# synthesizer-project/synference

Measured on AMD Instinct MI355X. Metric: posterior samples/sec (accepted, prior-box rejection included), higher is better.
Workload: dtype f32

## Files before the change

include/synference_hip.h:

```cpp
#ifndef SYNFERENCE_HIP_H
#define SYNFERENCE_HIP_H

#include <stddef.h>
#include <stdint.h>

#ifdef __cplusplus
extern "C" {
#endif

typedef struct sf_flow sf_flow;
typedef struct sf_opt sf_opt;

enum sf_status {
  SF_OK = 0,
  SF_ERR_INVALID = -1,
  SF_ERR_HIP = -2,
  SF_ERR_NO_DEVICE = -3,
  SF_ERR_STATE = -4
};

enum sf_kind { SF_MAF = 0, SF_NSF = 1, SF_NSF_AR = 2, SF_MAF_AR = 3 };

typedef struct sf_flow_desc {
  int32_t kind;
// ... 46 lines not shown

int sf_flow_log_prob_grad(sf_flow* f, const float* theta , const float* x, int64_t rows_per_x, int64_t B,
                          float* lp , float* dtheta , void* stream);

int sf_map_step(int64_t B, int64_t D, float* phi , float* exp_avg , float* exp_avg_sq ,
                float* theta , const float* lp , const float* g_theta , const float* lo ,
                const float* hi , float* best_theta , float* best_lp , float learning_rate,
                int64_t step, int save_best, void* stream);

int sf_flow_inverse_from_noise(sf_flow* f, const float* z , const float* x ,
                               int64_t B, float* theta , float* logdet ,
                               void* stream);
int sf_flow_inverse_from_noise_sampler(sf_flow* f, const float* z , const float* x , int64_t B,
                                       float* theta , void* stream);
int sf_set_sampler_fp32(int on);

int sf_flow_sample_round(sf_flow* f, const float* x , int64_t S,
                         const uint32_t* slots, int64_t slot_base, int64_t n_slots,
                         uint32_t attempt, int32_t attempts_per_slot, uint64_t seed, uint32_t stream_id,
                         const float* lo , const float* hi ,
                         float* out , uint32_t* rejected, uint32_t* n_rejected,
                         int32_t* n_drawn, void* stream);

int sf_flow_prepare_context(sf_flow* f, const float* x , int64_t M, void* stream);
int sf_flow_release_context(sf_flow* f);

int sf_flow_sample(sf_flow* f, const float* x , int64_t M, int64_t S,
                   const float* lo, const float* hi, uint64_t seed, int32_t max_attempts,
                   float* out , int32_t* n_drawn , int64_t* n_unfilled ,
                   void* stream);
// ... 188 lines not shown
```

synference_amd/_lib.py:

```python
from __future__ import annotations

import ctypes as C
import os
from pathlib import Path

_HERE = Path(__file__).resolve().parent
LIB_PATH = _HERE / "lib" / "libsynference_hip.so"

c_f32p = C.POINTER(C.c_float)
c_i32p = C.POINTER(C.c_int32)
c_u32p = C.POINTER(C.c_uint32)


class sf_flow_desc(C.Structure):
    _fields_ = [
        ("kind", C.c_int32), ("D", C.c_int32), ("C", C.c_int32), ("H", C.c_int32),
        ("T", C.c_int32), ("K", C.c_int32), ("NB", C.c_int32), ("scale_fn", C.c_int32),
        ("hidden_bf16", C.c_int32),
        ("tail_bound", C.c_float), ("min_bin_width", C.c_float), ("min_bin_height", C.c_float),
        ("min_derivative", C.c_float), ("maf_eps", C.c_float), ("lu_eps", C.c_float),
        ("theta_mean", c_f32p), ("theta_std", c_f32p), ("x_mean", c_f32p), ("x_std", c_f32p),
        ("perms", c_i32p), ("ar_slope", C.c_float),
    ]

# ... 40 lines not shown
                                    C.c_void_p, C.c_void_p, C.c_void_p]),
    "sf_scatter_empirical": (C.c_int, [C.c_void_p, C.c_int64, C.c_int32, C.POINTER(sf_noise_band), c_f32p, C.c_int64, C.c_int32,
                                       C.c_uint64, C.c_void_p, C.c_void_p, C.c_void_p]),
    "sf_apply_scalings": (C.c_int, [C.c_void_p, C.c_void_p, C.c_int64, C.c_int32, C.POINTER(sf_noise_band), c_f32p, C.c_int64,
                                    C.c_void_p, C.c_void_p, C.c_void_p]),
    "sf_pit_ranks": (C.c_int, [C.c_void_p, C.c_void_p, C.c_int64, C.c_int64, C.c_int32, C.c_void_p, C.c_void_p]),
    "sf_tarp_coverage": (C.c_int, [C.c_void_p, C.c_void_p, C.c_int64, C.c_int64, C.c_int32, C.c_void_p, C.c_int32, C.c_int32,
                                   C.c_int32, C.c_int32, C.c_uint64, C.c_void_p, C.c_void_p, C.c_void_p, C.c_void_p,
                                   C.c_void_p]),
    "sf_copy_to_host_f64": (C.c_int, [C.c_void_p, C.c_void_p, C.c_int64, C.c_void_p]),
    "sf_flow_packed16_size": (C.c_int64, [C.c_void_p]),
    "sf_flow_pack_table16": (C.c_int, [C.c_void_p, C.c_void_p, C.c_void_p, C.c_int64]),
    "sf_flow_packed16b_size": (C.c_int64, [C.c_void_p]),
    "sf_flow_inverse_from_noise_sampler": (C.c_int, [C.c_void_p, C.c_void_p, C.c_void_p, C.c_int64, C.c_void_p, C.c_void_p]),
    "sf_set_sampler_fp32": (C.c_int, [C.c_int]),
    "sf_flow_set_sample_row_offset": (C.c_int, [C.c_void_p, C.c_int64]),
    "sf_flow_train_path": (C.c_int, [C.c_void_p, C.c_int64, C.c_int]),
    "sf_flow_trainc_size": (C.c_int64, [C.c_void_p]),
    "sf_flow_trainc_grad_size": (C.c_int64, [C.c_void_p]),
    "sf_flow_cst_size": (C.c_int64, [C.c_void_p]),
    "sf_flow_trainc_table": (C.c_int, [C.c_void_p, C.c_void_p, C.c_void_p, C.c_int64, C.c_void_p, C.c_int64, C.c_void_p,
                                       C.c_void_p, C.c_int64]),
    "sf_flow_pack_table16b": (C.c_int, [C.c_void_p, C.c_void_p, C.c_int64]),
    "sf_flow_get_params": (C.c_int, [C.c_void_p, C.c_void_p, C.c_int64, C.c_int, C.c_void_p]),
    "sf_flow_prepare_context": (C.c_int, [C.c_void_p, C.c_void_p, C.c_int64, C.c_void_p]),
    "sf_flow_release_context": (C.c_int, [C.c_void_p]),
    "sf_flow_sample": (C.c_int, [C.c_void_p, C.c_void_p, C.c_int64, C.c_int64, C.c_void_p, C.c_void_p,
                                 C.c_uint64, C.c_int32, C.c_void_p, C.c_void_p, C.POINTER(C.c_int64),
                                 C.c_void_p]),
    "sf_flow_sample_slots": (C.c_int, [C.c_void_p, C.c_void_p, C.c_int64, C.c_int64, C.c_void_p, C.c_int64, C.c_void_p,
# ... 94 lines not shown
```

synference_amd/csrc/sf_api.hip:

```cpp
#include <hip/hip_runtime.h>

#include <chrono>
#include <cmath>
#include <cstdio>
#include <cstdlib>
#include <cstring>
#include <string>
#include <vector>

#include "sf_internal.h"
#include "sf_train.h"
#include "sf_nsf1.h"
#include "sf_nsfar.h"
#include "sf_nsfc.h"
#include "sf_trainc.h"

namespace {
thread_local std::string g_err;

int hip_fail(hipError_t e, const char* what) {
  return sf_fail(SF_ERR_HIP, std::string(what) + ": " + hipGetErrorString(e));
}
}

// ... 195 lines not shown
  add("o_wg0", v.o_wg[0]); add("o_bg0", v.o_bg[0]); add("o_w10", v.o_w1[0]); add("o_b10", v.o_b1[0]);
  add("o_w20", v.o_w2[0]); add("o_b20", v.o_b2[0]); add("o_wg1", v.o_wg[1]); add("o_bg1", v.o_bg[1]);
  add("o_w11", v.o_w1[1]); add("o_b11", v.o_b1[1]); add("o_w21", v.o_w2[1]); add("o_b21", v.o_b2[1]);
  add("o_wout", v.o_wout); add("o_bout", v.o_bout); add("o_lu", v.o_lu);
  add("c_pscale", v.c_pscale); add("c_pshift", v.c_pshift); add("c_tdim", v.c_tdim);
  add("c_xmean", v.c_xmean); add("c_xstd", v.c_xstd); add("c_dslot", v.c_dslot);
  add("nsf_split_sampler", f->L.nsfS.ok); add("trainc_ok", f->L.trc.ok); add("nsfc_ok", f->L.nsc.ok);
  add("inc_ok", v.inc_ok); add("hidden_bf16", v.hidden_bf16); add("tB_stride", v.tB_stride); add("n_parts", v.n_parts); add("part_max", v.part_max);
  add("n_params", f->L.n_params); add("n_packed", f->L.n_packed);
  {
    int R = 0, NV = 0;
    SfDev vv = v;
    vv.packed16 = reinterpret_cast<const float*>(1);
    sf_ctab_shape(vv, R, NV);
    add("ctab_floats_per_galaxy", (long)v.T * NV * R);
  }
  add("o16_w0", v.o16_w0); add("o16_wc", v.o16_wc); add("o16_b0", v.o16_b0); add("o16_wk0", v.o16_wk[0]);
  add("o16_wk1", v.o16_wk[1]); add("o16_bk0", v.o16_bk[0]); add("o16_bk1", v.o16_bk[1]); add("o16_hv", v.o16_hv);
  add("o16_hvb", v.o16_hvb); add("o16_wh", v.o16_wh); add("o16_bh", v.o16_bh); add("o16_wp", v.o16_wp); add("t16_a_tab", v.t16_a_tab);
  add("t16_a", v.t16_a); add("t16B_stride", v.t16B_stride); add("nP16", v.nP16); add("o16B_wk0", v.o16B_wk[0]); add("o16B_wk1", v.o16B_wk[1]);
  add("m16_ok", v.m16_ok); add("m16_span", v.m16_span); add("nT16", v.nT16); add("nC16", v.nC16); add("t16_stride", v.t16_stride);
  s += "\"g16_tile\": [";
  for (int i = 0; i < SF_DMAX; ++i) s += std::to_string(v.g16_tile[i]) + (i + 1 < SF_DMAX ? ", " : "], ");
  s += "\"g16_lo\": [";
  for (int i = 0; i < SF_DMAX; ++i) s += std::to_string(v.g16_lo[i]) + (i + 1 < SF_DMAX ? ", " : "], ");
  s += "\"g_kend\": [";
  for (int i = 0; i < SF_DMAX; ++i) s += std::to_string(v.g_kend[i]) + (i + 1 < SF_DMAX ? ", " : "], ");
  s += "\"g_lo\": [";
  for (int i = 0; i < SF_DMAX; ++i) s += std::to_string(v.g_lo[i]) + (i + 1 < SF_DMAX ? ", " : "], ");
  s += "\"g_tile\": [";
// ... 143 lines not shown
extern "C++" {
static int g_sampler_fp32 = -2;
void sf_sampler_fp32_set(int on) { g_sampler_fp32 = on < 0 ? -1 : (on ? 1 : 0); }
int sf_sampler_fp32_get() {
  if (g_sampler_fp32 == -2) { const char* e = std::getenv("SF_SAMPLER_FP32"); g_sampler_fp32 = (e && *e) ? (std::atoi(e) != 0 ? 1 : 0) : -1; }
  return g_sampler_fp32;
}
int sf_sampler_fp32_for(int kind) {
  const int g = sf_sampler_fp32_get();
  return g < 0 ? (kind == SF_MAF ? 1 : 0) : g;
}
}
int sf_set_sampler_fp32(int on) {
  sf_sampler_fp32_set(on);
  return SF_OK;
}

int sf_flow_train_path(const sf_flow* f, int64_t B, int want_dctx) {
  if (!f) return sf_fail(SF_ERR_INVALID, "null handle");
  if (f->nsf1) return 4;
  if (f->nsfar) return 5;
  if (B > 0 && sf_trainc_eligible(f->L, want_dctx != 0)) return sf_trainc_groups((long)B, &f->L.trc, f->L.dev.T);
  if (B > 0 && sf_nsfc_eligible(f->L, want_dctx != 0)) return 3;
  return 0;
}

static void seed_keys(uint64_t seed, uint32_t stream_id, uint32_t& k0, uint32_t& k1) {
  k0 = (uint32_t)(seed & 0xffffffffu);
  k1 = (uint32_t)(seed >> 32) ^ stream_id;
}
// ... 642 lines not shown
```

synference_amd/csrc/sf_internal.h:

```cpp
#pragma once
#include <hip/hip_runtime.h>
#include <stdint.h>

#include "sf_buf.h"
#include "sf_layout.h"
#include "sf_queue.h"

struct SfSampleArgsHost {
  const float* x = nullptr;
  const float* z_in = nullptr;
  long S = 1;
  const uint32_t* slots = nullptr;
  long slot_base = 0;
  long n_items = 0;
  uint32_t attempt = 0, k0 = 0, k1 = 0;
  unsigned long long rng_slot_offset = 0;
  int attempts_per_slot = 1;
  int log2_attempts = 0;
  const float* lo = nullptr;
  const float* hi = nullptr;
  float* out = nullptr;
  int out_f64 = 0;
  float* logdet_out = nullptr;
  uint32_t* rejected = nullptr;
// ... 33 lines not shown
void sf_sampler_fp32_set(int on);
int sf_sampler_fp32_get();
int sf_sampler_fp32_for(int kind);
void sf_ctab_shape(const SfDev& m, int& R, int& NV);
hipError_t sf_launch_ctab(const SfDev& m, const float* x, long M, float* tab, hipStream_t st);
hipError_t sf_launch_maf_ctab16(const SfDev& m, const float* x, long M, float* tab, hipStream_t st);
hipError_t sf_launch_maf_fuse16(const SfDev& m, hipStream_t st);
struct SfMaf16Plan {
  bool ok16 = false;
  bool sampler16 = false;
  bool fp32 = false;
  bool span = false;
  bool head_mfma = false;
  int dd = 0;
  bool fused = false;
};
SfMaf16Plan sf_maf16_plan(const SfDev& m);
hipError_t sf_launch_maf_find16_zin(const SfDev& m, const SfSampleArgsHost& a, hipStream_t st);
hipError_t sf_launch_pack(const float* flat, const int32_t* s1, const int32_t* s2, float* packed, long n,
                          hipStream_t st);
hipError_t sf_launch_pack_bf16(const float* flat, const int32_t* src, unsigned short* out, long n, hipStream_t st);
hipError_t sf_launch_pack_bf16_split(const float* flat, const int32_t* src, unsigned short* out, long n, hipStream_t st);
hipError_t sf_launch_fill_nan_rows(float* out, const uint32_t* slots, long n, int D, hipStream_t st, int out_f64 = 0);
hipError_t sf_launch_fill_i32(int32_t* p, long n, int32_t v, hipStream_t st);
hipError_t sf_launch_exclusive_scan_i32(const int32_t* cnt, int n, int32_t* offs, int32_t* total, hipStream_t st);
hipError_t sf_launch_account_window(const uint32_t* list, const uint32_t* best, long n, long S, uint32_t a_lo, uint32_t A,
                                    int32_t* n_drawn, int32_t* gal_acc, hipStream_t st);
hipError_t sf_launch_filter_survivors(uint32_t* list, unsigned int* n_surv, long S, const int32_t* gal_acc, float* out,
                                      int D, hipStream_t st, int out_f64 = 0);

#include <string>
#define SF_MAX_DEVICES 16
// ... 138 lines not shown
```

synference_amd/csrc/sf_maf16.hip:

```cpp
#include "sf_maf16_pass.h"

template <int NB, bool SPAN>
__global__ __launch_bounds__(256, 3) void k_maf_inv16(SfDev m, SfSampleArgsHost a) {
  const int lane = threadIdx.x & 63, wave = threadIdx.x >> 6;
  const int s = lane & 15, g4 = lane >> 4;
  const long item = ((long)blockIdx.x * 4 + wave) * 16 + s;
  const bool valid = item < a.n_items;
  const long it = valid ? item : a.n_items - 1;
  const SfItem16 I = sf_item16(m, a, it, g4);
  f32x4 u = I.u;
  const uint32_t slot = I.slot, att_mine = I.att;
  const long gal = I.gal, ps_idx = I.ps;
  const float* xr = a.x + gal * m.C;
  float logdet = 0.f;

  const float* ctg = (m.ctab && !a.z_in) ? m.ctab + (size_t)gal * m.T * m.ctab_R : nullptr;
  f32x4 ct0;
  if (!ctg) ct0 = sf_ctx_tile16(m, xr, 0, g4);

  const int NT = m.nT16;
  SfPass16 S;
#pragma unroll
  for (int k = 0; k < 3; ++k)
#pragma unroll
// ... 120 lines not shown
  static constexpr int oB_wk1 = entries * 512, B_stride = (NB * entries * 512 + 1023) / 1024 * 1024;
  static bool matches(const SfDev& m) {
    return m.nT16 == NT && m.o16_w0 == o_w0 && m.o16_b0 == o_b0 && m.o16_bk[0] == o_bk0 && (NB < 2 || m.o16_bk[1] == o_bk1) &&
           m.o16_hv == o_hv && m.o16_hvb == o_hvb && m.o16_wh == o_wh && m.o16_bh == o_bh && m.o16_wp == o_wp && m.t16_a_tab == a_tab &&
           m.o16B_wk[0] == 0 && (NB < 2 || m.o16B_wk[1] == oB_wk1) && m.t16B_stride == B_stride;
  }
  static __device__ __forceinline__ void apply(SfDev& m) {
    m.nT16 = NT; m.o16_w0 = o_w0; m.o16_b0 = o_b0; m.o16_bk[0] = o_bk0; m.o16_bk[1] = o_bk1; m.o16_hv = o_hv; m.o16_hvb = o_hvb;
    m.o16_wh = o_wh; m.o16_bh = o_bh; m.o16_wp = o_wp; m.t16_a_tab = a_tab; m.o16B_wk[0] = 0; m.o16B_wk[1] = oB_wk1; m.t16B_stride = B_stride;
  }
};

#ifndef SF_SAMP16_WG_FUSED
#define SF_SAMP16_WG_FUSED 4
#endif
template <int NB, bool SPAN, bool HM, int DD = 0, int PREC = 0>
__global__ __launch_bounds__(256, (SPAN ? 3 : (PREC == 2 ? SF_SAMP16_WG_FUSED : 4))) void k_maf_samp16(SfSamp16Args args_in) {
  static_assert(DD == 0 || (HM && !SPAN && DD >= 2 && DD <= 5), "unrolled passes: head tile, aligned placement, D <= 5");
  using HID = SfHid16<PREC>;
  constexpr int TPW = SF_SAMP16_TPW;
  constexpr int IPW = 64 * TPW;
  const int wave = threadIdx.x >> 6;
  unsigned int* ctrl = reinterpret_cast<unsigned int*>(
      sf_lds16 + (args_in.m.ctab ? args_in.m.t16_a_tab : args_in.m.t16_a) + HID::lds_floats(args_in.m, !SPAN));
  unsigned int pf;
  sf_q_begin<IPW>(args_in.a, ctrl, pf);
  float* ecb = reinterpret_cast<float*>(ctrl + SF_Q_WORDS(IPW));
  sf_ecb16_build<true>(ecb, args_in.m, args_in.a);
#ifdef SF_Q_STATS
  const unsigned long long qs_k0 = __builtin_amdgcn_s_memtime();
  unsigned long long qs_iters = 0, qs_last_work = 0;
  unsigned long long qs_ph[10] = {0, 0, 0, 0, 0, 0, 0, 0, 0, 0};
  if (threadIdx.x == 0) atomicMin(&args_in.a.q->stats[10], __builtin_amdgcn_s_memrealtime());
#endif
  for (;;) {
    const SfSamp16Args* ap;
    {
      auto kp = __builtin_amdgcn_kernarg_segment_ptr();
      asm volatile("" : "+s"(kp));
      ap = (const SfSamp16Args*)kp;
    }
    const SfDev& m_arg = ap->m;
    SfDev m_fix;
    if constexpr (DD > 0) { m_fix = m_arg; SfFix16<NB, DD>::apply(m_fix); }
    const SfDev& m = DD > 0 ? m_fix : m_arg;
    const SfSampleArgsHost& a = ap->a;
    const int lane = (threadIdx.x & 63) + sf_opaque_zero();
    const int s = lane & 15, g4 = lane >> 4;
#ifdef SF_Q_STATS
    const unsigned long long qs_t_top = __builtin_amdgcn_s_memrealtime();
#endif
    if (!sf_q_fetch<IPW, 64>(a, ctrl, pf)) {
#ifdef SF_Q_STATS
      if (threadIdx.x == 0) {
        for (int i = 0; i < 10; ++i) atomicAdd(&a.q->stats[14 + i], qs_ph[i]);
        atomicAdd(&a.q->stats[9], __builtin_amdgcn_s_memtime() - qs_k0);
        atomicMax(&a.q->stats[11], qs_iters);
        atomicMax(&a.q->stats[12], qs_last_work);
        atomicMax(&a.q->stats[13], __builtin_amdgcn_s_memrealtime());
      }
#endif
      break;
    }
#ifdef SF_Q_STATS
    if (a.qtrace && threadIdx.x == 0 && qs_iters < (2048u * 256u) / gridDim.x) {
      uint32_t* tr = a.qtrace + ((size_t)blockIdx.x * ((2048u * 256u) / gridDim.x) + qs_iters) * 4;
      tr[0] = (uint32_t)__builtin_amdgcn_s_memrealtime(); tr[1] = ctrl[0]; tr[2] = ctrl[1] | (ctrl[9] << 8);
    }
    ++qs_iters;
    const unsigned long long qs_t_fetch = __builtin_amdgcn_s_memrealtime();
    const int qs_o = ctrl[9] ? 5 : 0;
    qs_ph[qs_o + 0] += qs_t_fetch - qs_t_top;
    unsigned long long qs_t_mark = qs_t_fetch;
#endif
    const int NT = m.nT16;
    const unsigned int n_items = ctrl[0] << ctrl[1];
    f32x4 u_t[TPW];
    unsigned int g_t[TPW];
    f32x4& u_cur = u_t[0];
    unsigned int& gal_cur = g_t[0];
#pragma unroll
    for (int j = TPW - 1; j >= 0; --j) {
      const int wi = (j * 4 + wave) * 16 + s;
      const unsigned int n_ent = ctrl[0];
      const int lgA = (int)ctrl[1];
      const unsigned int e = (unsigned)wi >> lgA;
      const unsigned int ee = e < n_ent ? e : 0u;
      const uint32_t slot = ctrl[SF_Q_HDR + ee];
      const uint32_t att = ctrl[SF_Q_HDR + IPW + ee] + ((unsigned)wi & ((1u << lgA) - 1u));
      float z4[4];
      sf_normal4(a.k0, a.k1, (uint64_t)slot + a.rng_slot_offset, att, (uint32_t)g4, z4);
#pragma unroll
      for (int r = 0; r < 4; ++r) u_t[j][r] = (4 * g4 + r < m.D) ? z4[r] : 0.f;
      g_t[j] = slot / (uint32_t)a.S;
    }
    SfTiles16 tiles;
    if constexpr (DD == 0) tiles.pack(m);
    typename HID::State S;
    S.tab = DD > 0 ? true : m.ctab != nullptr;
    for (int t = m.T - 1; t >= 0; --t) {
      const int dsl = (int)m.cst[m.c_dslot + t * SF_DMAX + s];
      S.c0p = S.tab ? m.ctab + ((size_t)gal_cur * m.T + t) * m.ctab_R + (PREC == 2 ? m.nT16 * 16 : 0) : nullptr;
      if constexpr (PREC == 2) sf_pre16g_load<DD - 1>(S, g4);
      else if (HM && S.tab) sf_c0_prefetch(S, tiles.tile(2), g4);
#ifdef SF_Q_STATS
      { const unsigned long long n = __builtin_amdgcn_s_memrealtime(); qs_ph[qs_o + (t == m.T - 1 ? 1 : 3)] += n - qs_t_mark; qs_t_mark = n; }
#endif
      __syncthreads();
      sf_stage16<PREC, !SPAN>(m, t, S.tab ? m.t16_a_tab : m.t16_a, wave);
      __syncthreads();
#ifdef SF_Q_STATS
      { const unsigned long long n = __builtin_amdgcn_s_memrealtime(); qs_ph[qs_o + 2] += n - qs_t_mark; qs_t_mark = n; }
#endif
      const float* tp = sf_lds16;
      const void* tpB = sf_lds16 + (S.tab ? m.t16_a_tab : m.t16_a);
#pragma unroll 1
      for (int j = 0; j < TPW; ++j) {
        const bool tile_has_work = (unsigned)((j * 4 + wave) * 16) < n_items;
        if (tile_has_work) {
          if (j > 0) {
            S.c0p = S.tab ? m.ctab + ((size_t)gal_cur * m.T + t) * m.ctab_R + (PREC == 2 ? m.nT16 * 16 : 0) : nullptr;
            if constexpr (PREC == 2) sf_pre16g_load<DD - 1>(S, g4);
            else if (HM && S.tab) sf_c0_prefetch(S, tiles.tile(2), g4);
          }
          if (HM) S.hdone = sf_ld4(tp + m.o16_bh + g4 * 4);
          if constexpr (PREC == 2) {
            float* scr = (float*)tpB + HID::blk_floats(m) + wave * SF_G16_SCR + s * SF_G16_ROW;
            sf_transform16g<NB, DD>(m, tp, static_cast<const float*>(tpB), S, dsl, u_cur, scr, lane, g4);
          } else {
            S.xr = a.x + gal_cur * m.C;
            if constexpr (DD > 0) {
              sf_transform16s<HID, NB, DD>(m, tp, tpB, S, NT, dsl, u_cur, lane, g4);
            } else {
              HID::template clear<false, HM>(S);
#pragma unroll
              for (int r = 0; r < 4; ++r) S.ut[r] = 0.f;
              {
                const int sl = __builtin_amdgcn_readlane(dsl, 0);
                sf_pass16_deg1(m, tp, S.ut, sl, sf_slot16_own(u_cur, sl), g4);
              }
              for (int p = 2; p <= m.D; ++p) {
                const int sl = __builtin_amdgcn_readlane(dsl, p - 1);
// ... 6 lines not shown
        if (TPW > 1) {
          const f32x4 tu = u_t[0];
          const unsigned int tg = g_t[0];
#pragma unroll
          for (int q = 0; q + 1 < TPW; ++q) { u_t[q] = u_t[q + 1]; g_t[q] = g_t[q + 1]; }
          u_t[TPW - 1] = tu;
          g_t[TPW - 1] = tg;
        }
      }
    }
#ifdef SF_Q_STATS
    { const unsigned long long n = __builtin_amdgcn_s_memrealtime(); qs_ph[qs_o + 3] += n - qs_t_mark; qs_t_mark = n; }
#endif
#pragma unroll 1
    for (int j = 0; j < TPW; ++j) {
      const int wi = (j * 4 + wave) * 16 + s;
      const unsigned int n_ent = ctrl[0];
      const int lgA = (int)ctrl[1];
      const unsigned int e = (unsigned)wi >> lgA;
      const bool entry_ok = e < n_ent;
      const unsigned int ee = entry_ok ? e : 0u;
      const uint32_t slot = ctrl[SF_Q_HDR + ee];
      const uint32_t att_base = ctrl[SF_Q_HDR + IPW + ee];
      const uint32_t att = att_base + ((unsigned)wi & ((1u << lgA) - 1u));
      const bool valid = entry_ok && att < a.attempt_limit;
      float th[4];
      int tdc[4];
      const uint32_t acc16 = sf_accept16(sf_theta_box16(ecb, u_cur, g4, th, tdc), valid);
      const int A = 1 << lgA;
      int first, me;
      if (lgA <= 4) {
        const int grp0 = (s / A) * A;
        const uint32_t gmask = (acc16 >> grp0) & ((1u << A) - 1u);
        first = gmask ? (int)__builtin_ctz(gmask) : -1;
        me = s - grp0;
      } else {
        if ((threadIdx.x & 63) == 0) ctrl[20 + wave] = acc16 ? (unsigned)__builtin_ctz(acc16) : 16u;
        __syncthreads();
        const int gw0 = (int)(((e << lgA) >> 4) & 3u), gwn = A >> 4;
        first = -1;
#pragma unroll
        for (int w = 3; w >= 0; --w) {
          const unsigned int cw = ctrl[20 + w];
          if (w >= gw0 && w < gw0 + gwn && cw < 16u) first = (w - gw0) * 16 + (int)cw;
        }
        me = wi - (int)(e << lgA);
        if (TPW > 1) __syncthreads();
      }
      if (lgA == 0) {
        const int Dn = DD > 0 ? DD : m.D;
// ... 44 lines not shown
      }
      if (TPW > 1) {
        const f32x4 tu = u_t[0];
#pragma unroll
        for (int q = 0; q + 1 < TPW; ++q) u_t[q] = u_t[q + 1];
        u_t[TPW - 1] = tu;
      }
    }
#ifdef SF_Q_STATS
    qs_last_work = __builtin_amdgcn_s_memrealtime();
    qs_ph[qs_o + 4] += qs_last_work - qs_t_mark;
    if (a.qtrace && threadIdx.x == 0 && qs_iters <= (2048u * 256u) / gridDim.x)
      a.qtrace[((size_t)blockIdx.x * ((2048u * 256u) / gridDim.x) + qs_iters - 1) * 4 + 3] = (uint32_t)qs_last_work;
#endif
  }
}

template <int NB, int DD, int PREC = 0>
__global__ __launch_bounds__(256, 4) void k_maf_find16s(SfDev m, SfSampleArgsHost a) {
  using HID = SfHid16<PREC>;
  SfFix16<NB, DD>::apply(m);
  const int lane = threadIdx.x & 63, wave = threadIdx.x >> 6;
  const int s = lane & 15, g4 = lane >> 4;
  float* ecb = sf_lds16 + m.t16_a_tab + HID::lds_floats(m, true);
  sf_ecb16_build<false>(ecb, m, a);
  const int NT = m.nT16;
  f32x4 u_cur, u_oth;
  long gal_cur = 0, gal_oth = 0;
#pragma unroll
  for (int j = 1; j >= 0; --j) {
// ... 118 lines not shown
    if (m.g16_tile[p - 1] != p - 2) return 0;
  bool fits = false;
  if (m.NB == 1) fits = m.D == 3 ? SfFix16<1, 3>::matches(m) : (m.D == 4 ? SfFix16<1, 4>::matches(m) : SfFix16<1, 5>::matches(m));
  else if (m.NB == 2) fits = m.D == 3 ? SfFix16<2, 3>::matches(m) : (m.D == 4 ? SfFix16<2, 4>::matches(m) : SfFix16<2, 5>::matches(m));
  return fits ? m.D : 0;
}
SfMaf16Plan sf_maf16_plan(const SfDev& m) {
  SfMaf16Plan pl;
  pl.fp32 = sf_sampler_fp32_for(SF_MAF) != 0;
  pl.ok16 = m.kind == SF_MAF && m.m16_ok && !m.hidden_bf16 && m.packed16 != nullptr;
  pl.sampler16 = pl.ok16 && (m.packed16B != nullptr || pl.fp32);
  pl.span = m.m16_span != 0;
  pl.head_mfma = !m.m16_span && m.o16_wh >= 0;
  pl.dd = pl.head_mfma ? sf_maf16_seq_d(m) : 0;
  pl.fused = pl.dd > 0 && pl.fp32 && m.o16_wp >= 0 && m.ctab_R == 2 * m.nT16 * 16;
  return pl;
}

template <int NB, int DD, int PREC>
static hipError_t sf_launch_find16s(const SfDev& m, const SfSampleArgsHost& a, hipStream_t st) {
  static SfAttrCache attr;
  const size_t sh = ((size_t)m.t16_a_tab + (size_t)SfHid16<PREC>::lds_floats(m, true)) * sizeof(float) + 80 * sizeof(float);
  if (hipError_t e = sf_lds_optin16(k_maf_find16s<NB, DD, PREC>, attr); e != hipSuccess) return e;
  hipLaunchKernelGGL((k_maf_find16s<NB, DD, PREC>), dim3((unsigned)((a.n_items + 127) / 128)), dim3(256), sh, st, m, a);
  return hipGetLastError();
}

template <int NB, bool SPAN, bool HM, int PREC = 0>
__global__ __launch_bounds__(256, 3) void k_maf_inv16b(SfDev m, const float* __restrict__ z, const float* __restrict__ x,
                                                       long n, float* __restrict__ out) {
  using HID = SfHid16<PREC>;
// ... 128 lines not shown
  }
}
hipError_t sf_launch_maf_fuse16(const SfDev& m, hipStream_t st) {
  hipLaunchKernelGGL(k_maf_fuse16, dim3((unsigned)m.T), dim3(256), 0, st, m);
  return hipGetLastError();
}
hipError_t sf_launch_maf_ctab16(const SfDev& m, const float* x, long M, float* tab, hipStream_t st) {
  hipLaunchKernelGGL(k_maf_ctab16, dim3((unsigned)((M + 63) / 64), (unsigned)m.T), dim3(256), 0, st, m, x, M, tab);
  return hipGetLastError();
}

bool sf_maf16_enabled(const SfDev& m, const SfSampleArgsHost& a) {
  return sf_maf16_plan(m).ok16 && (a.attempts_per_slot <= 16 || a.best != nullptr);
}

static int sf_resident_blocks16(const void* fn, size_t sh, int cap) {
  int dev = 0, cus = 256, per = cap;
  if (hipGetDevice(&dev) == hipSuccess) {
    hipDeviceProp_t pr;
    if (hipGetDeviceProperties(&pr, dev) == hipSuccess && pr.multiProcessorCount > 0) cus = pr.multiProcessorCount;
  }
  int occ = 0;
  if (hipOccupancyMaxActiveBlocksPerMultiprocessor(&occ, fn, 256, sh) == hipSuccess && occ > 0) per = occ < cap ? occ : cap;
  return cus * per;
}

template <int NB, bool SPAN, bool HM, int DD, int PREC>
static hipError_t sf_launch16q_p(const SfDev& m, const SfSampleArgsHost& a, hipStream_t st) {
  static SfAttrCache attr;
  static SfResidentCache rcache;
  const size_t sh = ((size_t)(m.ctab ? m.t16_a_tab : m.t16_a) + (size_t)SfHid16<PREC>::lds_floats(m, !SPAN)) * sizeof(float) +
                    (SF_Q_WORDS(64 * SF_SAMP16_TPW) + 96) * sizeof(unsigned int);
  if (sh > 160 * 1024) return hipErrorInvalidValue;
  if (hipError_t e = sf_lds_optin16(k_maf_samp16<NB, SPAN, HM, DD, PREC>, attr); e != hipSuccess) return e;
  int resident = 0, cur_dev = 0;
  (void)hipGetDevice(&cur_dev);
  if (!rcache.get(cur_dev, sh, resident)) {
    resident = sf_resident_blocks16((const void*)k_maf_samp16<NB, SPAN, HM, DD, PREC>, sh, SPAN ? 3 : (PREC == 2 ? SF_SAMP16_WG_FUSED : 4));
    rcache.put(cur_dev, sh, resident);
  }
  long grid = (a.n_items + 64 * SF_SAMP16_TPW - 1) / (64 * SF_SAMP16_TPW);
  if (grid > resident) grid = resident;
  SfSamp16Args args;
  args.m = m;
  args.a = a;
  hipLaunchKernelGGL((k_maf_samp16<NB, SPAN, HM, DD, PREC>), dim3((unsigned)grid), dim3(256), sh, st, args);
  return hipGetLastError();
}
template <int NB, bool SPAN, bool HM, int DD>
static hipError_t sf_launch16q(const SfDev& m, const SfSampleArgsHost& a, const SfMaf16Plan& pl, hipStream_t st) {
  if constexpr (DD > 0) {
    if (pl.fused) return sf_launch16q_p<NB, SPAN, HM, DD, 2>(m, a, st);
  }
  if (pl.fp32) return sf_launch16q_p<NB, SPAN, HM, DD, 1>(m, a, st);
  if (!m.packed16B) return hipErrorInvalidValue;
  return sf_launch16q_p<NB, SPAN, HM, DD, 0>(m, a, st);
}
template <int NB, bool SPAN>
static hipError_t sf_launch16(const SfDev& m, const SfSampleArgsHost& a, hipStream_t st) {
  static SfAttrCache attr;
  const size_t sh = (size_t)m.t16_stride * sizeof(float);
  if (hipError_t e = sf_lds_optin16(k_maf_inv16<NB, SPAN>, attr); e != hipSuccess) return e;
  const long per_block = 4L * 16;
  hipLaunchKernelGGL((k_maf_inv16<NB, SPAN>), dim3((unsigned)((a.n_items + per_block - 1) / per_block)), dim3(256), sh, st, m, a);
  return hipGetLastError();
// ... 23 lines not shown
```

synference_amd/csrc/sf_maf16_pass.h:

```cpp
#pragma once
#include <hip/hip_runtime.h>

#include <type_traits>

#include "sf_device.h"
#include "sf_internal.h"
#include "sf_rng.h"

typedef float f32x4 __attribute__((ext_vector_type(4)));
typedef float f32x2 __attribute__((ext_vector_type(2)));
#define SF_MFMA16(a, b, c) __builtin_amdgcn_mfma_f32_16x16x4f32((a), (b), (c), 0, 0, 0)

__device__ __forceinline__ float sf_sum4groups(float v) {
  v += __shfl_xor(v, 16, 64);
  v += __shfl_xor(v, 32, 64);
  return v;
}
__device__ __forceinline__ f32x4 sf_mma16(float4 w, const f32x4& in, f32x4 acc) {
  acc = SF_MFMA16(w.x, in[0], acc);
  acc = SF_MFMA16(w.y, in[1], acc);
  acc = SF_MFMA16(w.z, in[2], acc);
  acc = SF_MFMA16(w.w, in[3], acc);
  return acc;
}
// ... 651 lines not shown
    const int NT = m.nT16, nb = m.NB < 2 ? m.NB : 2;
    const int per = CP ? NT * (NT + 1) / 2 : NT * NT;
    constexpr int K0 = PREC == 2 ? 1 : 0;
    float4* __restrict__ dF = d4 + (a_floats >> 2);
    for (int e = __builtin_amdgcn_readfirstlane(wave); e < (nb - K0) * per; e += 4) {
      const int k = K0 + (e >= per ? 1 : 0), ee = e - (k - K0) * per;
      int src_blk = ee;
      if (CP) {
        const int ot = ee >= 6 ? 3 : (ee >= 3 ? 2 : (ee >= 1 ? 1 : 0));
        src_blk = ot * NT + (ee - ot * (ot + 1) / 2);
      }
      const int owk = k ? m.o16_wk[1] : m.o16_wk[0];
      const float4* g = sa + ((owk >> 2) + src_blk * 64) + lane_;
      __builtin_amdgcn_global_load_lds((const void*)g, (void __attribute__((address_space(3)))*)(dF + e * 64), 16, 0, 0);
    }
  }
  __builtin_amdgcn_s_waitcnt(0x0f70);
}

struct SfHid16Plain {
  using State = SfPass16;
  template <int OT, int NB, bool CP, bool HM>
  static __device__ __forceinline__ void pass(const SfDev& m, const float* tp, const void*, State& S, int NT, int sl, float u_sl,
                                              int lane, int g4, int) {
    sf_pass16<OT, NB>(m, tp, S, NT, sl, u_sl, lane, g4);
  }
  template <int LO, int HI, int NB>
  static __device__ __forceinline__ void span(const SfDev& m, const float* tp, const void*, State& S, int NT, int sl, float u_sl,
                                              int lane, int g4) {
    sf_pass16_span<LO, HI, NB>(m, tp, S, NT, sl, u_sl, lane, g4);
// ... 109 lines not shown
```

synference_amd/csrc/sf_queue.h:

```cpp
#pragma once
#include <hip/hip_runtime.h>
#include <stdint.h>

struct SfQueue {
  unsigned int dense_next; unsigned int _p0[31];
  unsigned int head;       unsigned int _p1[31];
  unsigned int reserve;    unsigned int _p2[31];
  unsigned int resolved;   unsigned int _p3[31];
  unsigned int n_surv;     unsigned int dropped;
  unsigned int _p4[30];
  unsigned int error;      unsigned int _p5[31];
  unsigned int rej0;       unsigned int _p6[31];
  unsigned long long evals; unsigned int _p7[30];
  unsigned long long stats[24];
};

#define SF_Q_SPIN_TICKS 1500000000ull
#define SF_Q_SPIN_ITERS 4000000u

#define SF_Q_HDR 24
#define SF_Q_WORDS(IPW) (SF_Q_HDR + 5 * (IPW))

__device__ __forceinline__ unsigned int sf_q_ld(const unsigned int* p) {
  return __hip_atomic_load(p, __ATOMIC_RELAXED, __HIP_MEMORY_SCOPE_AGENT);
}

#ifdef __HIPCC__
#ifdef SF_Q_STATS
#define SF_QS_T() __builtin_amdgcn_s_memtime()
#define SF_QS_ADD(i, v) do { if (threadIdx.x == 0) atomicAdd(&a.q->stats[i], (unsigned long long)(v)); } while (0)
#else
#define SF_QS_T() 0ull
#define SF_QS_ADD(i, v) do { } while (0)
#endif
template <int IPW, int AMAX, class Args>
__device__ __forceinline__ bool sf_q_fetch(const Args& a, unsigned int* ctrl, unsigned int& pf) {
  const unsigned long long qs_t0 = SF_QS_T();
  __syncthreads();
  const unsigned long long qs_t1 = SF_QS_T();
  if (threadIdx.x < 64) {
    const int lane = threadIdx.x;
    SfQueue* q = a.q;
    unsigned int* w_slot = ctrl + SF_Q_HDR;
    unsigned int* w_att = w_slot + IPW;
    const unsigned int* p_slot = w_att + IPW;
    const unsigned int* p_att = p_slot + IPW;
    const unsigned int* s_slot = p_att + IPW;
    constexpr unsigned int KEEP = IPW / AMAX;
    const unsigned int sc = ctrl[3];
    if (sc) {
      unsigned int pos = 0;
      if (lane == 0) pos = atomicAdd(&q->n_surv, sc);
      pos = __builtin_amdgcn_readfirstlane(pos);
      for (unsigned int i = lane; i < sc; i += 64) {
        if (pos + i < a.n_total) a.rejected[pos + i] = s_slot[i];
        else atomicExch(&q->error, 3u);
// ... 6 lines not shown
    }
    unsigned int dcur = ctrl[7], dend = ctrl[8], dense_done = ctrl[9];
    if (!dense_done && n >= (unsigned)IPW && dcur >= dend) {
      if (__shfl(pf, 0, 64) >= a.n_total) dense_done = 1u;
    }
#pragma unroll 1
    for (int seg = 0; seg < 2; ++seg) {
      if (dense_done || n >= (unsigned)IPW) break;
      if (dcur >= dend) {
        const unsigned int nb = __shfl(pf, 0, 64);
        if (nb >= a.n_total) {
          dense_done = 1u;
          break;
        }
        dcur = nb;
        dend = a.n_total - nb < (unsigned)IPW ? a.n_total : nb + (unsigned)IPW;
        if (lane == 0) pf = atomicAdd(&q->dense_next, (unsigned)IPW);
      }
      const unsigned int want = (unsigned)IPW - n;
      const unsigned int nd = dend - dcur < want ? dend - dcur : want;
      for (unsigned int i = lane; i < nd; i += 64) {
        unsigned int sl;
        if (a.slots) {
          unsigned int pos = dcur + i;
          if (a.list_mul) {
            const unsigned int msk = (1u << a.list_log2) - 1u;
            do { pos = (pos * a.list_mul) & msk; } while (pos >= a.n_total);
          }
          sl = a.slots[pos];
        } else if (a.dense_G) {
          const unsigned int idx = dcur + i, S_ = (unsigned int)a.S, M_ = a.n_total / S_;
          const unsigned int per_block = a.dense_G * S_, b = idx / per_block, j = idx - b * per_block;
// ... 105 lines not shown
          mn = ot < mn ? ot : mn;
        }
        const unsigned int amax_now = mn < 4u ? 2u : (mn < (unsigned)AMAX ? mn : (unsigned)AMAX);
        while ((2u << lg) * n <= (unsigned)IPW && (2u << lg) <= amax_now) ++lg;
      }
      if (lane == 0) ctrl[10] = nt;
    }
    if (lane == 0) {
      ctrl[0] = n; ctrl[1] = lg; ctrl[2] = 0; ctrl[3] = 0;
      ctrl[7] = dcur; ctrl[8] = dend; ctrl[9] = dense_done;
    }
    SF_QS_ADD(dense_done ? 7 : 6, 1);
    SF_QS_ADD(8, n);
  }
  const unsigned long long qs_t2 = SF_QS_T();
  __syncthreads();
  SF_QS_ADD(0, qs_t1 - qs_t0);
  SF_QS_ADD(1, qs_t2 - qs_t1);
  SF_QS_ADD(2, SF_QS_T() - qs_t2);
  return ctrl[0] != 0u;
}

template <int IPW, class Args>
__device__ __forceinline__ void sf_q_begin(const Args& a, unsigned int* ctrl, unsigned int& pf) {
  if (threadIdx.x < SF_Q_HDR) ctrl[threadIdx.x] = 0u;
  pf = 0u;
  if (threadIdx.x == 0) pf = atomicAdd(&a.q->dense_next, (unsigned)IPW);
}
#endif
```

Baseline: 1.089 billion.

## Add LDS-resident weight sampler kernel with per-wave work queues

Adds a 1024-thread, one-workgroup-per-CU sampler variant. It stages every transform's weight images into LDS once at kernel start, so the per-transform global-to-LDS restaging and its two workgroup barriers go away. The work queue gains a wave scope, letting each wave fetch and refill its own items with wave barriers instead of __syncthreads. Speculative acceptance is now resolved across a wave's two tiles. The path is chosen automatically when the images fit in 160 KiB and there are enough items to fill the resident grid. The cost is lower occupancy (one large block per CU) and more LDS pressure.

Measured after the change: 789.4 million. -27.5%, worse.

```diff
diff --git a/include/synference_hip.h b/include/synference_hip.h
--- a/include/synference_hip.h
+++ b/include/synference_hip.h
@@ -84,6 +84,7 @@
 int sf_flow_inverse_from_noise_sampler(sf_flow* f, const float* z , const float* x , int64_t B,
                                        float* theta , void* stream);
 int sf_set_sampler_fp32(int on);
+int sf_set_sampler_resident(int mode);
 
 int sf_flow_sample_round(sf_flow* f, const float* x , int64_t S,
                          const uint32_t* slots, int64_t slot_base, int64_t n_slots,
diff --git a/synference_amd/_lib.py b/synference_amd/_lib.py
--- a/synference_amd/_lib.py
+++ b/synference_amd/_lib.py
@@ -78,6 +78,7 @@
     "sf_flow_packed16b_size": (C.c_int64, [C.c_void_p]),
     "sf_flow_inverse_from_noise_sampler": (C.c_int, [C.c_void_p, C.c_void_p, C.c_void_p, C.c_int64, C.c_void_p, C.c_void_p]),
     "sf_set_sampler_fp32": (C.c_int, [C.c_int]),
+    "sf_set_sampler_resident": (C.c_int, [C.c_int]),
     "sf_flow_set_sample_row_offset": (C.c_int, [C.c_void_p, C.c_int64]),
     "sf_flow_train_path": (C.c_int, [C.c_void_p, C.c_int64, C.c_int]),
     "sf_flow_trainc_size": (C.c_int64, [C.c_void_p]),
diff --git a/synference_amd/csrc/sf_api.hip b/synference_amd/csrc/sf_api.hip
--- a/synference_amd/csrc/sf_api.hip
+++ b/synference_amd/csrc/sf_api.hip
@@ -233,6 +233,11 @@
     vv.packed16 = reinterpret_cast<const float*>(1);
     sf_ctab_shape(vv, R, NV);
     add("ctab_floats_per_galaxy", (long)v.T * NV * R);
+    vv.ctab = reinterpret_cast<const float*>(1);
+    vv.ctab_R = R; vv.ctab_NV = NV;
+    const SfMaf16Plan pl = sf_maf16_plan(vv);
+    add("sampler_resident", pl.resident ? 1 : 0);
+    add("sampler_resident_bytes", pl.fused ? (long)sf_maf16_resident_bytes(vv) : 0);
   }
   add("o16_w0", v.o16_w0); add("o16_wc", v.o16_wc); add("o16_b0", v.o16_b0); add("o16_wk0", v.o16_wk[0]);
   add("o16_wk1", v.o16_wk[1]); add("o16_bk0", v.o16_bk[0]); add("o16_bk1", v.o16_bk[1]); add("o16_hv", v.o16_hv);
@@ -406,6 +411,13 @@
 int sf_set_sampler_fp32(int on) {
   sf_sampler_fp32_set(on);
   return SF_OK;
+}
+static int g_sampler_resident = -1;
+extern "C++" int sf_sampler_resident_get() { return g_sampler_resident; }
+int sf_set_sampler_resident(int mode) {
+  const int prev = g_sampler_resident;
+  g_sampler_resident = mode < 0 ? -1 : (mode ? 1 : 0);
+  return prev;
 }
 
 int sf_flow_train_path(const sf_flow* f, int64_t B, int want_dctx) {
diff --git a/synference_amd/csrc/sf_internal.h b/synference_amd/csrc/sf_internal.h
--- a/synference_amd/csrc/sf_internal.h
+++ b/synference_amd/csrc/sf_internal.h
@@ -71,8 +71,11 @@
   bool head_mfma = false;
   int dd = 0;
   bool fused = false;
+  bool resident = false;
 };
 SfMaf16Plan sf_maf16_plan(const SfDev& m);
+size_t sf_maf16_resident_bytes(const SfDev& m);
+int sf_sampler_resident_get();
 hipError_t sf_launch_maf_find16_zin(const SfDev& m, const SfSampleArgsHost& a, hipStream_t st);
 hipError_t sf_launch_pack(const float* flat, const int32_t* s1, const int32_t* s2, float* packed, long n,
                           hipStream_t st);
diff --git a/synference_amd/csrc/sf_maf16.hip b/synference_amd/csrc/sf_maf16.hip
--- a/synference_amd/csrc/sf_maf16.hip
+++ b/synference_amd/csrc/sf_maf16.hip
@@ -158,19 +158,54 @@
 #ifndef SF_SAMP16_WG_FUSED
 #define SF_SAMP16_WG_FUSED 4
 #endif
-template <int NB, bool SPAN, bool HM, int DD = 0, int PREC = 0>
-__global__ __launch_bounds__(256, (SPAN ? 3 : (PREC == 2 ? SF_SAMP16_WG_FUSED : 4))) void k_maf_samp16(SfSamp16Args args_in) {
+#ifndef SF_SAMP16R_TPW
+#define SF_SAMP16R_TPW 2
+#endif
+template <int NB, int DD>
+struct SfRes16 {
+  using F = SfFix16<NB, DD>;
+  static constexpr int WAVES = 16, TPW = SF_SAMP16R_TPW, IPW = 16 * TPW;
+  static constexpr int RANGE = 128;
+  static constexpr int a_floats = F::a_tab - F::o_b0;
+  static constexpr int blk_floats = NB >= 2 ? F::NT * (F::NT + 1) / 2 * 256 : 0;
+  static constexpr int per = a_floats + blk_floats;
+  static constexpr int wave_words = SF_Q_WORDS(IPW) + SF_G16_SCR;
+  static constexpr int o_ecb = WAVES * wave_words;
+  static constexpr int o_img = (o_ecb + 96 + 255) / 256 * 256;
+  static_assert(a_floats % 256 == 0 && blk_floats % 256 == 0 && wave_words % 4 == 0, "1 KiB copy units, 16-byte rows");
+  static_assert(o_img >= F::o_b0, "tp = base_t - o16_b0 stays inside the LDS window");
+  static constexpr size_t bytes(int T) { return ((size_t)o_img + (size_t)T * per) * sizeof(float); }
+};
+
+template <int NB, bool SPAN, bool HM, int DD, int PREC, bool RES>
+__device__ __forceinline__ void sf_samp16_worker(const SfSamp16Args& args_in) {
   static_assert(DD == 0 || (HM && !SPAN && DD >= 2 && DD <= 5), "unrolled passes: head tile, aligned placement, D <= 5");
+  static_assert(!RES || (PREC == 2 && DD >= 3), "resident images: the fused fp32 form of the unrolled kernels");
   using HID = SfHid16<PREC>;
-  constexpr int TPW = SF_SAMP16_TPW;
-  constexpr int IPW = 64 * TPW;
+  using RL = SfRes16<NB, (RES ? DD : 5)>;
+  constexpr int TPW = RES ? RL::TPW : SF_SAMP16_TPW;
+  constexpr int IPW = (RES ? 16 : 64) * TPW;
+  constexpr int AMAX = RES ? 16 * TPW : 64;
+  constexpr int QSCOPE = RES ? SF_Q_WAVE : SF_Q_WORKGROUP;
+  constexpr int QRANGE = RES ? RL::RANGE : IPW;
   const int wave = threadIdx.x >> 6;
-  unsigned int* ctrl = reinterpret_cast<unsigned int*>(
-      sf_lds16 + (args_in.m.ctab ? args_in.m.t16_a_tab : args_in.m.t16_a) + HID::lds_floats(args_in.m, !SPAN));
+  unsigned int* ctrl;
+  float* ecb;
+  if constexpr (RES) {
+    ctrl = reinterpret_cast<unsigned int*>(sf_lds16 + wave * RL::wave_words);
+    ecb = sf_lds16 + RL::o_ecb;
+  } else {
+    ctrl = reinterpret_cast<unsigned int*>(
+        sf_lds16 + (args_in.m.ctab ? args_in.m.t16_a_tab : args_in.m.t16_a) + HID::lds_floats(args_in.m, !SPAN));
+    ecb = reinterpret_cast<float*>(ctrl + SF_Q_WORDS(IPW));
+  }
   unsigned int pf;
-  sf_q_begin<IPW>(args_in.a, ctrl, pf);
-  float* ecb = reinterpret_cast<float*>(ctrl + SF_Q_WORDS(IPW));
+  sf_q_begin<IPW, QSCOPE, QRANGE>(args_in.a, ctrl, pf);
   sf_ecb16_build<true>(ecb, args_in.m, args_in.a);
+  if constexpr (RES) {
+    sf_stage16r<RL>(args_in.m, wave);
+    __syncthreads();
+  }
 #ifdef SF_Q_STATS
   const unsigned long long qs_k0 = __builtin_amdgcn_s_memtime();
   unsigned long long qs_iters = 0, qs_last_work = 0;
@@ -194,7 +229,7 @@
 #ifdef SF_Q_STATS
     const unsigned long long qs_t_top = __builtin_amdgcn_s_memrealtime();
 #endif
-    if (!sf_q_fetch<IPW, 64>(a, ctrl, pf)) {
+    if (!sf_q_fetch<IPW, AMAX, QSCOPE, QRANGE>(a, ctrl, pf)) {
 #ifdef SF_Q_STATS
       if (threadIdx.x == 0) {
         for (int i = 0; i < 10; ++i) atomicAdd(&a.q->stats[14 + i], qs_ph[i]);
@@ -225,7 +260,7 @@
     unsigned int& gal_cur = g_t[0];
 #pragma unroll
     for (int j = TPW - 1; j >= 0; --j) {
-      const int wi = (j * 4 + wave) * 16 + s;
+      const int wi = (RES ? j : j * 4 + wave) * 16 + s;
       const unsigned int n_ent = ctrl[0];
       const int lgA = (int)ctrl[1];
       const unsigned int e = (unsigned)wi >> lgA;
@@ -250,17 +285,22 @@
 #ifdef SF_Q_STATS
       { const unsigned long long n = __builtin_amdgcn_s_memrealtime(); qs_ph[qs_o + (t == m.T - 1 ? 1 : 3)] += n - qs_t_mark; qs_t_mark = n; }
 #endif
-      __syncthreads();
-      sf_stage16<PREC, !SPAN>(m, t, S.tab ? m.t16_a_tab : m.t16_a, wave);
-      __syncthreads();
+      const float* tp;
+      if constexpr (RES) {
+        tp = sf_lds16 + (RL::o_img - RL::F::o_b0) + t * RL::per;
+      } else {
+        __syncthreads();
+        sf_stage16<PREC, !SPAN>(m, t, S.tab ? m.t16_a_tab : m.t16_a, wave);
+        __syncthreads();
 #ifdef SF_Q_STATS
-      { const unsigned long long n = __builtin_amdgcn_s_memrealtime(); qs_ph[qs_o + 2] += n - qs_t_mark; qs_t_mark = n; }
-#endif
-      const float* tp = sf_lds16;
-      const void* tpB = sf_lds16 + (S.tab ? m.t16_a_tab : m.t16_a);
+        { const unsigned long long n = __builtin_amdgcn_s_memrealtime(); qs_ph[qs_o + 2] += n - qs_t_mark; qs_t_mark = n; }
+#endif
+        tp = sf_lds16;
+      }
+      const void* tpB = (RES ? tp : sf_lds16) + (S.tab ? m.t16_a_tab : m.t16_a);
 #pragma unroll 1
       for (int j = 0; j < TPW; ++j) {
-        const bool tile_has_work = (unsigned)((j * 4 + wave) * 16) < n_items;
+        const bool tile_has_work = (unsigned)((RES ? j : j * 4 + wave) * 16) < n_items;
         if (tile_has_work) {
           if (j > 0) {
             S.c0p = S.tab ? m.ctab + ((size_t)gal_cur * m.T + t) * m.ctab_R + (PREC == 2 ? m.nT16 * 16 : 0) : nullptr;
@@ -269,7 +309,8 @@
           }
           if (HM) S.hdone = sf_ld4(tp + m.o16_bh + g4 * 4);
           if constexpr (PREC == 2) {
-            float* scr = (float*)tpB + HID::blk_floats(m) + wave * SF_G16_SCR + s * SF_G16_ROW;
+            float* scr = (RES ? reinterpret_cast<float*>(ctrl) + SF_Q_WORDS(IPW) : (float*)tpB + HID::blk_floats(m) + wave * SF_G16_SCR) +
+                         s * SF_G16_ROW;
             sf_transform16g<NB, DD>(m, tp, static_cast<const float*>(tpB), S, dsl, u_cur, scr, lane, g4);
           } else {
             S.xr = a.x + gal_cur * m.C;
@@ -306,7 +347,7 @@
 #endif
 #pragma unroll 1
     for (int j = 0; j < TPW; ++j) {
-      const int wi = (j * 4 + wave) * 16 + s;
+      const int wi = (RES ? j : j * 4 + wave) * 16 + s;
       const unsigned int n_ent = ctrl[0];
       const int lgA = (int)ctrl[1];
       const unsigned int e = (unsigned)wi >> lgA;
@@ -326,6 +367,15 @@
         const uint32_t gmask = (acc16 >> grp0) & ((1u << A) - 1u);
         first = gmask ? (int)__builtin_ctz(gmask) : -1;
         me = s - grp0;
+      } else if constexpr (RES) {
+        static_assert(TPW <= 2, "a speculation group spans the wave's two tiles at most");
+        const int wo = wi ^ 16;
+        float tho[4];
+        int tdo[4];
+        const uint32_t acc_o = sf_accept16(sf_theta_box16(ecb, u_t[TPW - 1], g4, tho, tdo), entry_ok && att_base + (uint32_t)wo < a.attempt_limit);
+        const uint32_t acc32 = j == 0 ? (acc16 | (acc_o << 16)) : (acc_o | (acc16 << 16));
+        first = acc32 ? (int)__builtin_ctz(acc32) : -1;
+        me = wi;
       } else {
         if ((threadIdx.x & 63) == 0) ctrl[20 + wave] = acc16 ? (unsigned)__builtin_ctz(acc16) : 16u;
         __syncthreads();
@@ -400,6 +450,14 @@
       a.qtrace[((size_t)blockIdx.x * ((2048u * 256u) / gridDim.x) + qs_iters - 1) * 4 + 3] = (uint32_t)qs_last_work;
 #endif
   }
+}
+template <int NB, bool SPAN, bool HM, int DD = 0, int PREC = 0>
+__global__ __launch_bounds__(256, (SPAN ? 3 : (PREC == 2 ? SF_SAMP16_WG_FUSED : 4))) void k_maf_samp16(SfSamp16Args args_in) {
+  sf_samp16_worker<NB, SPAN, HM, DD, PREC, false>(args_in);
+}
+template <int NB, int DD>
+__global__ __launch_bounds__(1024, 1) void k_maf_samp16r(SfSamp16Args args_in) {
+  sf_samp16_worker<NB, false, true, DD, 2, true>(args_in);
 }
 
 template <int NB, int DD, int PREC = 0>
@@ -548,7 +606,17 @@
   pl.head_mfma = !m.m16_span && m.o16_wh >= 0;
   pl.dd = pl.head_mfma ? sf_maf16_seq_d(m) : 0;
   pl.fused = pl.dd > 0 && pl.fp32 && m.o16_wp >= 0 && m.ctab_R == 2 * m.nT16 * 16;
+  const size_t rb = pl.fused ? sf_maf16_resident_bytes(m) : 0;
+  pl.resident = rb > 0 && rb <= 160 * 1024;
   return pl;
+}
+size_t sf_maf16_resident_bytes(const SfDev& m) {
+  size_t b = 0;
+  (void)sf_visit_unrolled16(m.NB, m.D, [&](auto nb, auto dd) {
+    b = SfRes16<nb(), dd()>::bytes(m.T);
+    return hipSuccess;
+  });
+  return b;
 }
 
 template <int NB, int DD, int PREC>
@@ -707,14 +775,14 @@
   return sf_maf16_plan(m).ok16 && (a.attempts_per_slot <= 16 || a.best != nullptr);
 }
 
-static int sf_resident_blocks16(const void* fn, size_t sh, int cap) {
+static int sf_resident_blocks16(const void* fn, size_t sh, int cap, int threads = 256) {
   int dev = 0, cus = 256, per = cap;
   if (hipGetDevice(&dev) == hipSuccess) {
     hipDeviceProp_t pr;
     if (hipGetDeviceProperties(&pr, dev) == hipSuccess && pr.multiProcessorCount > 0) cus = pr.multiProcessorCount;
   }
   int occ = 0;
-  if (hipOccupancyMaxActiveBlocksPerMultiprocessor(&occ, fn, 256, sh) == hipSuccess && occ > 0) per = occ < cap ? occ : cap;
+  if (hipOccupancyMaxActiveBlocksPerMultiprocessor(&occ, fn, threads, sh) == hipSuccess && occ > 0) per = occ < cap ? occ : cap;
   return cus * per;
 }
 
@@ -740,8 +808,40 @@
   hipLaunchKernelGGL((k_maf_samp16<NB, SPAN, HM, DD, PREC>), dim3((unsigned)grid), dim3(256), sh, st, args);
   return hipGetLastError();
 }
+template <int NB, int DD>
+static hipError_t sf_launch16r(const SfDev& m, const SfSampleArgsHost& a, hipStream_t st) {
+  using RL = SfRes16<NB, DD>;
+  static SfAttrCache attr;
+  static SfResidentCache rcache;
+  const int mode = sf_sampler_resident_get();
+  if (mode == 0) return hipErrorNotReady;
+  const size_t sh = RL::bytes(m.T);
+  if (sh > 160 * 1024) return hipErrorInvalidValue;
+  if (hipError_t e = sf_lds_optin16(k_maf_samp16r<NB, DD>, attr); e != hipSuccess) return e;
+  int resident = 0, cur_dev = 0;
+  (void)hipGetDevice(&cur_dev);
+  if (!rcache.get(cur_dev, sh, resident)) {
+    resident = sf_resident_blocks16((const void*)k_maf_samp16r<NB, DD>, sh, 1, 1024);
+    rcache.put(cur_dev, sh, resident);
+  }
+  const long per_wg = (long)RL::WAVES * RL::IPW;
+  if (mode < 0 && a.n_items < (long)resident * per_wg) return hipErrorNotReady;
+  long grid = (a.n_items + per_wg - 1) / per_wg;
+  if (grid > resident) grid = resident;
+  SfSamp16Args args;
+  args.m = m;
+  args.a = a;
+  hipLaunchKernelGGL((k_maf_samp16r<NB, DD>), dim3((unsigned)grid), dim3(1024), sh, st, args);
+  return hipGetLastError();
+}
 template <int NB, bool SPAN, bool HM, int DD>
 static hipError_t sf_launch16q(const SfDev& m, const SfSampleArgsHost& a, const SfMaf16Plan& pl, hipStream_t st) {
+  if constexpr (DD >= 3) {
+    if (pl.resident) {
+      const hipError_t e = sf_launch16r<NB, DD>(m, a, st);
+      if (e != hipErrorNotReady) return e;
+    }
+  }
   if constexpr (DD > 0) {
     if (pl.fused) return sf_launch16q_p<NB, SPAN, HM, DD, 2>(m, a, st);
   }
diff --git a/synference_amd/csrc/sf_maf16_pass.h b/synference_amd/csrc/sf_maf16_pass.h
--- a/synference_amd/csrc/sf_maf16_pass.h
+++ b/synference_amd/csrc/sf_maf16_pass.h
@@ -689,6 +689,25 @@
       const float4* g = sa + ((owk >> 2) + src_blk * 64) + lane_;
       __builtin_amdgcn_global_load_lds((const void*)g, (void __attribute__((address_space(3)))*)(dF + e * 64), 16, 0, 0);
     }
+  }
+  __builtin_amdgcn_s_waitcnt(0x0f70);
+}
+template <class RL>
+__device__ __forceinline__ void sf_stage16r(const SfDev& m, int wave) {
+  constexpr int NT = RL::F::NT, UA = RL::a_floats >> 8, UN = RL::per >> 8;
+  const int lane_ = threadIdx.x & 63;
+  const int owk = m.o16_wk[1];
+  for (int i = __builtin_amdgcn_readfirstlane(wave); i < m.T * UN; i += RL::WAVES) {
+    const int t = i / UN, e = i - t * UN;
+    int src4 = (RL::F::o_b0 >> 2) + e * 64;
+    if (e >= UA) {
+      const int ee = e - UA;
+      const int ot = ee >= 6 ? 3 : (ee >= 3 ? 2 : (ee >= 1 ? 1 : 0));
+      src4 = (owk >> 2) + (ot * NT + (ee - ot * (ot + 1) / 2)) * 64;
+    }
+    const float4* g = reinterpret_cast<const float4*>(m.packed16 + (size_t)t * m.t16_stride) + src4 + lane_;
+    float* l = sf_lds16 + RL::o_img + t * RL::per + e * 256;
+    __builtin_amdgcn_global_load_lds((const void*)g, (void __attribute__((address_space(3)))*)l, 16, 0, 0);
   }
   __builtin_amdgcn_s_waitcnt(0x0f70);
 }
diff --git a/synference_amd/csrc/sf_queue.h b/synference_amd/csrc/sf_queue.h
--- a/synference_amd/csrc/sf_queue.h
+++ b/synference_amd/csrc/sf_queue.h
@@ -25,7 +25,21 @@
   return __hip_atomic_load(p, __ATOMIC_RELAXED, __HIP_MEMORY_SCOPE_AGENT);
 }
 
+#define SF_Q_WORKGROUP 0
+#define SF_Q_WAVE 1
+
 #ifdef __HIPCC__
+template <int SCOPE>
+__device__ __forceinline__ void sf_q_sync() {
+  if constexpr (SCOPE == SF_Q_WAVE) {
+    __builtin_amdgcn_fence(__ATOMIC_RELEASE, "wavefront");
+    __builtin_amdgcn_s_waitcnt(0xc07f);
+    __builtin_amdgcn_wave_barrier();
+    __builtin_amdgcn_fence(__ATOMIC_ACQUIRE, "wavefront");
+  } else {
+    __syncthreads();
+  }
+}
 #ifdef SF_Q_STATS
 #define SF_QS_T() __builtin_amdgcn_s_memtime()
 #define SF_QS_ADD(i, v) do { if (threadIdx.x == 0) atomicAdd(&a.q->stats[i], (unsigned long long)(v)); } while (0)
@@ -33,13 +47,14 @@
 #define SF_QS_T() 0ull
 #define SF_QS_ADD(i, v) do { } while (0)
 #endif
-template <int IPW, int AMAX, class Args>
+template <int IPW, int AMAX, int SCOPE = SF_Q_WORKGROUP, int RANGE = IPW, class Args>
 __device__ __forceinline__ bool sf_q_fetch(const Args& a, unsigned int* ctrl, unsigned int& pf) {
+  static_assert(RANGE >= IPW && IPW >= AMAX, "a top-up spans two ranges at most; a speculation group fits the worker's items");
   const unsigned long long qs_t0 = SF_QS_T();
-  __syncthreads();
+  sf_q_sync<SCOPE>();
   const unsigned long long qs_t1 = SF_QS_T();
-  if (threadIdx.x < 64) {
-    const int lane = threadIdx.x;
+  if (SCOPE == SF_Q_WAVE || threadIdx.x < 64) {
+    const int lane = SCOPE == SF_Q_WAVE ? (int)(threadIdx.x & 63u) : (int)threadIdx.x;
     SfQueue* q = a.q;
     unsigned int* w_slot = ctrl + SF_Q_HDR;
     unsigned int* w_att = w_slot + IPW;
@@ -76,8 +91,8 @@
           break;
         }
         dcur = nb;
-        dend = a.n_total - nb < (unsigned)IPW ? a.n_total : nb + (unsigned)IPW;
-        if (lane == 0) pf = atomicAdd(&q->dense_next, (unsigned)IPW);
+        dend = a.n_total - nb < (unsigned)RANGE ? a.n_total : nb + (unsigned)RANGE;
+        if (lane == 0) pf = atomicAdd(&q->dense_next, (unsigned)RANGE);
       }
       const unsigned int want = (unsigned)IPW - n;
       const unsigned int nd = dend - dcur < want ? dend - dcur : want;
@@ -213,17 +228,18 @@
     SF_QS_ADD(8, n);
   }
   const unsigned long long qs_t2 = SF_QS_T();
-  __syncthreads();
+  sf_q_sync<SCOPE>();
   SF_QS_ADD(0, qs_t1 - qs_t0);
   SF_QS_ADD(1, qs_t2 - qs_t1);
   SF_QS_ADD(2, SF_QS_T() - qs_t2);
   return ctrl[0] != 0u;
 }
 
-template <int IPW, class Args>
+template <int IPW, int SCOPE = SF_Q_WORKGROUP, int RANGE = IPW, class Args>
 __device__ __forceinline__ void sf_q_begin(const Args& a, unsigned int* ctrl, unsigned int& pf) {
-  if (threadIdx.x < SF_Q_HDR) ctrl[threadIdx.x] = 0u;
+  const unsigned int l = SCOPE == SF_Q_WAVE ? (threadIdx.x & 63u) : threadIdx.x;
+  if (l < SF_Q_HDR) ctrl[l] = 0u;
   pf = 0u;
-  if (threadIdx.x == 0) pf = atomicAdd(&a.q->dense_next, (unsigned)IPW);
+  if (l == 0) pf = atomicAdd(&a.q->dense_next, (unsigned)RANGE);
 }
 #endif
```
